# datavisorgaohui/kube-scheduler-simulator

Hardware: AMD Instinct MI355X
Metric: pod x node filter+score evals/sec (pods scheduled/sec in extra) (higher is better)
Workload: dtype int64/f64; 1 GPU; C2: 5000 nodes x 10000 pods, default profile, sequential, pct=100; nodes=5000, pods=10000, parallelism=scenario x1, percentage_of_nodes_to_score=100

## Files before the change

kube-scheduler-simulator_amd/csrc/kss_simple.cuh:

```cuda
#pragma once
#include "kss_fastmath.cuh"
#include "kss_sched.cuh"

namespace kss {

#define KSS_GLOBAL __attribute__((address_space(1)))
template <class T>
__device__ __forceinline__ KSS_GLOBAL T* gp(T* p) {
  return (KSS_GLOBAL T*)p;
}

template <class T>
__device__ __forceinline__ T ld_ag(const T* p) {
  return __hip_atomic_load(gp(p), __ATOMIC_RELAXED, __HIP_MEMORY_SCOPE_AGENT);
}
template <class T>
__device__ __forceinline__ T ld_ag(KSS_GLOBAL const T* p) {
  return __hip_atomic_load(p, __ATOMIC_RELAXED, __HIP_MEMORY_SCOPE_AGENT);
}
template <class T>
__device__ __forceinline__ void st_ag(T* p, T v) {
  __hip_atomic_store(gp(p), v, __ATOMIC_RELAXED, __HIP_MEMORY_SCOPE_AGENT);
}

// ... 1655 lines not shown
      if (sp && tid == 0) sp[1] = wall_clock64();
      best = wave_max_key(best, kb, c.node_base);
      if (sp && tid == 0) sp[2] = wall_clock64();
    } else {
      if (k >= k0) {
        if (keys) {
          for (int s = tid; s < own; s += nt) {
            const SVal e = cv_get(L, s == sub_s ? sub_h : s);
            const long long key = simple_key(prof, e, scored, max_tt, rtt, max_na, rna, (uint32_t)(c.node_base + lo + s));
            bool kept = true;
            if (WIN && wcs >= 0) {
              const int n = lo + s, seg = (n >= wsl ? 0 : W) + w;
              kept = seg < wcs || (seg == wcs && n < wd);
            }
            best = (e.f == 0 && kept && key > best) ? key : best;
          }
        }
        if (sp && tid == 0) sp[1] = wall_clock64();
        long long b[1] = {best};
        const int op[1] = {OP_MAX};
        block_red(H, parity, b, op);
        parity ^= 1;
        best = b[0];
        if (sp && tid == 0) sp[2] = wall_clock64();
      }
    }
    cand = best ? (int)(0xFFFFFFFFu - (uint32_t)(unsigned long long)best) - c.node_base - lo : -1;
    const SPod& qn = L.ring[(k + 1) % RING];
    const int sln = (k + 1) % RING;
    if constexpr (WIN) {
      if (k >= k0 && wcs >= 0) {
        wss = wcs % W;
        if (w == wss) wsx = wd;
        wsl = win_start(wss, wd);
      }
      uint32_t u[12];
      if (k + 1 < k1) {
        if constexpr (PW) simple_pass_a_pw_win<DEF>(prof, qn, pk, L, sln, own, pwv, cand, lo, wsl, u);
        else simple_pass_a_win<DEF>(prof, qn, pk, L, sln, own, cand, lo, wsl, u);
      } else {
#pragma unroll
        for (int i = 0; i < 12; i++) u[i] = 0;
      }
      if (sp && tid == 0) sp[3] = wall_clock64();
      if (!simple_sync_win<PW>(H, parity, best, u, W, w, ++epoch, gran, X, err, per, c.node_base, lo, own, pk, k >= k0, L,
                               kb, k_find, wsl, pwv, R, wd, wcs, sp, prefetch_idle))
        return;
    } else if constexpr (PW) {
      uint32_t u[6];
      if (k + 1 < k1) {
        simple_pass_a_pw<DEF>(prof, qn, pk, L, sln, own, pwv, cand, u);
      } else {
#pragma unroll
        for (int i = 0; i < 6; i++) u[i] = 0;
      }
      if (sp && tid == 0) sp[3] = wall_clock64();
      if (!simple_sync_pw(H, parity, best, u, W, w, ++epoch, gran, X, err, per, c.node_base, lo, own, pk, k >= k0, L, kb,
                          R, sp, prefetch_idle))
        return;
    } else {
      if (k + 1 < k1) {
        simple_pass_a<DEF>(prof, qn, pk, L, sln, own, cand, st);
      } else {
#pragma unroll
        for (int i = 0; i < 6; i++) st[i] = 0;
      }
      if (sp && tid == 0) sp[3] = wall_clock64();
      if (!simple_sync(H, parity, best, st, W, w, ++epoch, gran, X, err, per, c.node_base, kb, R, sp)) return;
    }
    if (sp && tid == 0) sp[5] = wall_clock64();
    if (k >= k0) {
      const long long K = R[0];
      const int x = K ? (int)(0xFFFFFFFFu - (uint32_t)(unsigned long long)K) - c.node_base : -1;
      const bool won = x >= lo && x < hi;
      sub_s = won ? x - lo : -1;
      sub_h = PW ? cap + (won ? (x - lo) / max(pwv, 1) : 0) : cap;
      if (!PW && !WIN && won && tid < 64) simple_commit_lanes(L, pk, x - lo, tid);
    }
    if (!defer_out) ring_store();
    if (k >= k0 && w == X.w_off && tid == out_tid) {
      const long long K = R[0];
      const int x = K ? (int)(0xFFFFFFFFu - (uint32_t)(unsigned long long)K) - c.node_base : -1;
      pend.chosen = K ? x + c.node_base : -1;
      pend.n_feasible = (int)nf;
      pend.scored = (K && scored) ? 1 : 0;
      pend.status = pk.status != 0 ? (pk.status == KSS_PF_ERROR ? 3 : 2) : (nf == 0 ? 1 : 0);
      pend.best_total = pend.scored ? (int64_t)((unsigned long long)K >> 32) : 0;
      pend_k = k;
      if (!defer_out) store_pending();
    }
    if (sp && tid == 0) sp[6] = wall_clock64();
  }
  if (tid == out_tid) store_pending();
  if constexpr (WIN) {
    if (X.n <= 1) {
      if (cursor && w == wss && tid == 0) st_ag(cursor, (int32_t)wsx);
    } else {
      const size_t co = 2 * (size_t)W * SXW_VALS + 2 * SXW_E2;
      ++epoch;
      if (w == wss && tid == 0) xpub(X, gran, co, ((unsigned long long)epoch << 32) | (uint32_t)wsx);
      if (w == X.w_off && tid == 0) {
        long long t0_ = 0;
        for (unsigned spins = 0;; ++spins) {
          const unsigned long long g = __hip_atomic_load(gran + co, __ATOMIC_RELAXED, __HIP_MEMORY_SCOPE_AGENT);
          if ((g >> 32) == epoch) {
            if (cursor) st_ag(cursor, (int32_t)(uint32_t)g);
            break;
          }
          if (spin_expired(spins, t0_)) {
            H.abort = 1;
            err_raise(err, 1);
            break;
          }
          spin_pause();
        }
      }
    }
  }
  __syncthreads();
  if (WIN && X.n > 1 && H.abort) return;
  for (int s = tid; s < own; s += nt) {
    const int n = lo + s;
#pragma unroll
    for (int r = 0; r < 3; r++) st_ag(&c.requested[(size_t)r * N + n], (int64_t)L.r64[(3 + r) * cap + s]);
    st_ag(&c.nonzero[n], (int64_t)L.r64[6 * cap + s]);
    st_ag(&c.nonzero[N + n], (int64_t)L.r64[7 * cap + s]);
    st_ag(&c.pod_count[n], L.r32[s]);
    for (int i = 0; i < L.nsc; i++) st_ag(&c.requested[(size_t)(3 + i) * N + n], L.sc[(size_t)(L.nsc + i) * cap + s]);
  }
  handoff_release();
}

constexpr int SXF_VALS = 4;
constexpr int SXF_LOADS = 8;
constexpr int SXF_MAX_E = 64 * SXF_LOADS / SXF_VALS;
static_assert(PW_LANES < 256, "granule 1 packs a wave's feasible counts in 8 bits");

__host__ __device__ constexpr int flat_entry(int gl, int per, int N, int nwave) {
  const int sh = gl / per, lo = sh * per;
  const int own = (N - lo < per ? N - lo : per);
  const int pwv = (own + nwave - 1) / nwave;
  return sh * nwave + (gl - lo) / pwv;
}
__host__ __device__ constexpr uint32_t flat_entry_range(int e, int per, int N, int W, int nwave) {
  const int sh = e / nwave, v = e - sh * nwave;
  if (sh >= W) return 0u;
  const int lo = sh * per;
  const int own = N - lo < 0 ? 0 : (N - lo < per ? N - lo : per);
  const int pwv = (own + nwave - 1) / nwave;
  const int a = v * pwv < own ? v * pwv : own, b = a + pwv < own ? a + pwv : own;
  return ((uint32_t)(lo + a) << 8) | (uint32_t)(b - a);
}
__host__ __device__ constexpr bool flat_range_holds(uint32_t r, int gl) {
  return (uint32_t)(gl - (int)(r >> 8)) < (r & 0xFFu);
}
__host__ __device__ constexpr bool flat_ranges_agree(int N, int W, int nwave) {
  const int per = (N + W - 1) / W;
  for (int gl = 0; gl < N; gl++)
    for (int e = 0; e < W * nwave; e++)
      if (flat_range_holds(flat_entry_range(e, per, N, W, nwave), gl) != (e == flat_entry(gl, per, N, nwave))) return false;
  for (int e = 0; e < W * nwave; e++)
    if (flat_range_holds(flat_entry_range(e, per, N, W, nwave), -1)) return false;
  return true;
}
static_assert(flat_ranges_agree(377, 3, 2) && flat_ranges_agree(378, 3, 2) && flat_ranges_agree(3, 3, 3) &&
                  flat_ranges_agree(10, 2, 3) && flat_ranges_agree(9, 2, 3) && flat_ranges_agree(5, 4, 2) &&
                  flat_ranges_agree(128, 64, 2) && flat_ranges_agree(1007, 2, 8),
              "flat_entry_range: the lanes' ranges are flat_entry's mapping");
static_assert(flat_entry(376, 126, 377, 2) == 5 && flat_entry(314, 126, 377, 2) == 4 && flat_entry(315, 126, 377, 2) == 5 &&
                  flat_entry(251, 126, 377, 2) == 3 && flat_entry(252, 126, 377, 2) == 4,
              "flat_entry: last shard one node short");
static_assert(flat_entry(0, 1, 3, 3) == 0 && flat_entry(1, 1, 3, 3) == 3 && flat_entry(2, 1, 3, 3) == 6,
              "flat_entry: shards of one node");
static_assert(flat_entry(1, 5, 10, 3) == 0 && flat_entry(2, 5, 10, 3) == 1 && flat_entry(4, 5, 10, 3) == 2 &&
                  flat_entry(5, 5, 10, 3) == 3 && flat_entry(9, 5, 10, 3) == 5,
              "flat_entry: own not divisible by nwave");
static_assert(flat_entry(8, 5, 9, 3) == 4 && flat_entry(6, 5, 9, 3) == 3, "flat_entry: short last shard, empty last wave");

template <typename Idle>
__device__ __forceinline__ bool simple_sync_flat(SimpleHdr& H, int& parity, long long wbest, uint32_t (&u)[6], int W,
                                                 int w, unsigned epoch, unsigned long long* gran, const XPeers& X,
                                                 int* err, int node_base, int kb, const uint32_t (&er)[SXF_LOADS],
                                                 long long (&R)[4], KSS_GLOBAL unsigned long long* sp, Idle&& idle) {
  wave_red_stats_pw(u);
  const int lane = threadIdx.x & 63, wave = threadIdx.x >> 6, nw = blockDim.x >> 6;
  const int E = W * nw;
  const unsigned long long tag = (unsigned long long)epoch << 32;
  if (sp && threadIdx.x == 0) sp[7] = wall_clock64();
  if (lane < SXF_VALS) {
    uint32_t x = key_compress(wbest, kb, node_base);
    x = lane == 1 ? (u[0] | (u[1] << 8) | (u[3] << 16) | (u[4] << 24)) : x;
    x = lane == 2 ? u[2] : x;
    x = lane == 3 ? u[5] : x;
    xpub(X, gran, ((size_t)(epoch & 1) * E + (size_t)w * nw + wave) * SXF_VALS + lane, tag | x);
  }
  if (sp && threadIdx.x == 0) sp[4] = wall_clock64();
  if (sp && (threadIdx.x == 64 || threadIdx.x == 128)) sp[9 + (threadIdx.x >> 6)] = wall_clock64();
  if (lane == 0) H.red[parity][wave][0] = wbest;
  lds_barrier();
  if (sp && threadIdx.x == 0) sp[8] = wall_clock64();
  idle();
  if (wave == 0) {
    if (sp && lane == 0) sp[15] = wall_clock64();
    const int G = SXF_VALS * E, nld = (G + 63) >> 6;
    const unsigned long long* base = gran + (size_t)(epoch & 1) * G;
    uint32_t got[SXF_LOADS];
    bool done = false;
    long long t0_ = 0;
    for (unsigned spins = 0;; ++spins) {
      bool ok = true;
      unsigned long long g[SXF_LOADS];
#pragma unroll
      for (int i = 0; i < SXF_LOADS; i++) {
        g[i] = tag;
        if (i < nld) {
          const int idx = i * 64 + lane;
          g[i] = __hip_atomic_load(base + (idx < G ? idx : 0), __ATOMIC_RELAXED, __HIP_MEMORY_SCOPE_AGENT);
        }
      }
#pragma unroll
      for (int i = 0; i < SXF_LOADS; i++) {
        ok &= (g[i] >> 32) == epoch;
        got[i] = i * 64 + lane < G ? (uint32_t)g[i] : 0u;
      }
      if (__all(ok)) {
        done = true;
        break;
      }
      if (spin_expired(spins, t0_)) break;
      spin_pause();
    }
    if (!done) {
      if (lane == 0) {
        H.abort = 1;
        err_raise(err, 1);
      }
    } else {
      const int field = lane & 3;
      uint32_t k = 0;
#pragma unroll
      for (int i = 0; i < SXF_LOADS; i++) k = max(k, got[i]);
      k = field == 0 ? k : 0u;
#define KSS_KSTEP(CTRL, ROWS) k = max(k, (uint32_t)__builtin_amdgcn_update_dpp(0, (int)k, CTRL, ROWS, 0xF, false))
      KSS_KSTEP(0xB1, 0xF);
      KSS_KSTEP(0x4E, 0xF);
      KSS_KSTEP(0x141, 0xF);
      KSS_KSTEP(0x140, 0xF);
      KSS_KSTEP(0x142, 0xA);
      KSS_KSTEP(0x143, 0xC);
#undef KSS_KSTEP
      k = (uint32_t)__builtin_amdgcn_readlane((int)k, 63);
      const long long best = key_expand(k, kb, node_base);
      const int gl = k ? (int)(((1u << kb) - 1u) - (k & ((1u << kb) - 1u))) : -1;
      uint32_t nf = 0, tt = 0, na = 0;
#pragma unroll
      for (int i = 0; i < SXF_LOADS; i++) {
        const bool h1 = flat_range_holds(er[i], gl);
        const uint32_t v = got[i];
        const uint32_t b = h1 ? v >> 16 : v;
        nf += field == 1 ? (b & 0xFFu) : 0u;
        tt = max(tt, field == 1 ? ((b >> 8) & 0xFFu) : 0u);
        na = max(na, (field == 2 && !h1) || (field == 3 && h1) ? v : 0u);
      }
#define KSS_FSTEP(CTRL, ROWS)                                                                      \
  {                                                                                                \
    const uint32_t a_ = (uint32_t)__builtin_amdgcn_update_dpp(0, (int)nf, CTRL, ROWS, 0xF, false); \
    const uint32_t b_ = (uint32_t)__builtin_amdgcn_update_dpp(0, (int)tt, CTRL, ROWS, 0xF, false); \
    const uint32_t c_ = (uint32_t)__builtin_amdgcn_update_dpp(0, (int)na, CTRL, ROWS, 0xF, false); \
    nf += a_;                                                                                      \
    tt = max(tt, b_);                                                                              \
    na = max(na, c_);                                                                              \
  }
      KSS_FSTEP(0xB1, 0xF)
      KSS_FSTEP(0x4E, 0xF)
      KSS_FSTEP(0x141, 0xF)
      KSS_FSTEP(0x140, 0xF)
      KSS_FSTEP(0x142, 0xA)
      KSS_FSTEP(0x143, 0xC)
#undef KSS_FSTEP
      if (lane == 63) {
        H.res[0] = best;
        H.res[1] = nf;
        H.res[2] = tt;
        H.res[3] = na;
      }
    }
  }
  parity ^= 1;
  lds_barrier();
  if (H.abort) return false;
#pragma unroll
  for (int i = 0; i < 4; i++) R[i] = H.res[i];
  return true;
}

template <bool FLAT>
__device__ __forceinline__ void simple_schedule_tab(DevCluster c, const SPod* __restrict__ spods,
                                                    const uint32_t* __restrict__ stat, int k0, int k1, int n_pods,
                                                    int32_t* chosen, PodMeta* meta, int W, int w, int cap,
                                                    unsigned long long* gran, const XPeers& X, unsigned epoch0, int* err,
                                                    unsigned long long* stamps, long long* smem, int n_shapes) {
  constexpr kss_profile prof = default_profile_c();
  constexpr int PD = 3;
  constexpr int NQ = (int)(sizeof(SPod) / 16);
  const int tid = threadIdx.x, nt = blockDim.x;
  SimpleHdr& H = *reinterpret_cast<SimpleHdr*>(smem);
  const SimpleShard L = shard_view(reinterpret_cast<uint8_t*>(smem) + sizeof(SimpleHdr), cap, 0);
  const ShapeTab TB = shape_tab_view(reinterpret_cast<uint8_t*>(smem), cap, n_shapes);
  const size_t N = (size_t)c.N;
  const int per = (c.N + W - 1) / W;
  const int lo = min(c.N, w * per), hi = min(c.N, lo + per), own = hi - lo;
  if (k1 <= k0) return;
  const int nwave = nt >> 6, lane = tid & 63, wv = tid >> 6;
  const int pwv = (own + nwave - 1) / nwave;
  const int s = wv * pwv + lane;
  const bool mine = lane < pwv && s < own;
  handoff_acquire();
  for (int i = tid; i < own; i += nt) {
    const int n = lo + i;
#pragma unroll
    for (int k = 0; k < 3; k++) {
      const int64_t A = c.alloc[k * N + n];
      L.r64[k * cap + i] = (double)A;
      L.r64[(3 + k) * cap + i] = (double)ld_ag(&c.requested[k * N + n]);
      L.inv[k * cap + i] = A > 0 ? 1.0 / (double)A : 0.0;
    }
    L.r64[6 * cap + i] = (double)ld_ag(&c.nonzero[n]);
    L.r64[7 * cap + i] = (double)ld_ag(&c.nonzero[N + n]);
    L.r32[i] = ld_ag(&c.pod_count[n]);
    L.r32[cap + i] = c.allowed_pods[n];
    for (int d = 0; d < PD && k0 + d < k1; d++) L.st[((k0 + d) % RING) * cap + i] = ld_ag(&stat[(size_t)d * N + lo + i]);
  }
  for (int i = tid; i < min(k1 - k0, PD) * NQ; i += nt) {
    const int j = k0 + i / NQ;
    reinterpret_cast<uint4*>(L.ring + j % RING)[i % NQ] = reinterpret_cast<const uint4*>(spods + j)[i % NQ];
  }
  for (int j = tid; j < n_shapes; j += nt) {
    const SPod& r = spods[min(max(spods[j].shape_rep, 0), n_pods - 1)];
    SShape d;
#pragma unroll
    for (int i = 0; i < 3; i++) d.fit_req[i] = r.fit_req[i];
#pragma unroll
    for (int i = 0; i < 2; i++) {
      d.snz[i] = r.snz[i];
      d.sreq[i] = r.sreq[i];
    }
    d.flags = r.flags;
    d.pad = 0;
    uint64_t dw[SSHAPE_WORDS];
    __builtin_memcpy(dw, &d, sizeof(SShape));
#pragma unroll
    for (int i = 0; i < SSHAPE_WORDS; i++) TB.shp[i * n_shapes + j] = dw[i];
  }
  if (tid == 0) H.abort = 0;
  __syncthreads();
  if (mine) {
    const DynRow r = shard_row(L, s);
    for (int j = 0; j < n_shapes; j++) TB.T[j * TB.ts + s] = shape_pack(dyn_eval_def(shape_get(TB, j), 0u, r));
  }
  __syncthreads();

  KSS_GLOBAL const uint32_t* gstat = gp(stat);
  KSS_GLOBAL const uint4* gspod = gp(reinterpret_cast<const uint4*>(spods));
  KSS_GLOBAL unsigned long long* gstamps = gp(stamps);
  long long R[4] = {0, 0, 0, 0};
  constexpr int out_tid = 64;
  PodMeta pend{};
  int pend_k = -1;
  auto store_pending = [&]() {
    if (pend_k < 0) return;
    if (chosen) gp(chosen)[pend_k] = pend.chosen;
    if (meta) {
      KSS_GLOBAL PodMeta* mm = gp(meta) + pend_k;
      mm->chosen = pend.chosen;
      mm->n_feasible = pend.n_feasible;
      mm->scored = pend.scored;
      mm->status = pend.status;
      mm->best_total = pend.best_total;
    }
    pend_k = -1;
  };
  int parity = 0;
  unsigned epoch = epoch0;
  const int kb = key_bits(prof, c.N);
  const int pf_w0 = nwave >= 3 ? nwave - 1 : 1;
  const bool pf_wave = __builtin_amdgcn_readfirstlane(tid >> 6) >= pf_w0;
  uint4 pfq = make_uint4(0, 0, 0, 0);
  uint32_t pfw[PF_MAX];
#pragma unroll
  for (int j = 0; j < PF_MAX; j++) pfw[j] = 0;
  const int pf_lane = tid - 64 * pf_w0, pf_n = nt - 64 * pf_w0;
  const int pf_per = (own + pf_n - 1) / pf_n;
  const int idle_n = 64 * (nwave - 1), jobs = nwave * n_shapes;
  const int job0 = tid - 64;
  const int v0 = job0 >= 0 ? job0 / n_shapes : 0, j0 = job0 >= 0 ? job0 % n_shapes : 0;
  int ck = 0, cn = min(max(L.ring[k0 % RING].shape, 0), n_shapes - 1), cnn = 0;
  uint32_t er[SXF_LOADS] = {};
  if constexpr (FLAT) {
#pragma unroll
    for (int i = 0; i < SXF_LOADS; i++) er[i] = flat_entry_range(i * 16 + (lane >> 2), per, c.N, W, nwave);
  }
  for (int k = k0 - 1; k < k1; k++) {
    KSS_GLOBAL unsigned long long* sp = (stamps && k >= k0 && k - k0 < KSS_NSTAMP_PODS / 2)
                                            ? gstamps + (size_t)w * 8 * KSS_NSTAMP_PODS + (size_t)(k - k0) * 16
                                            : nullptr;
    if (sp && tid == 0) sp[0] = wall_clock64();
    if (sp && tid == 64) sp[9] = wall_clock64();
    const SPod& pk = L.ring[(k + RING) % RING];
    const SPod& qn = L.ring[(k + 1) % RING];
    const int slk = (k + RING) % RING, sln = (k + 1) % RING;
    if (k + 2 < k1) cnn = min(max(L.ring[(k + 2) % RING].shape, 0), n_shapes - 1);
    const bool pf_on = pf_wave && k >= k0 && k + PD < k1 && own > 0;
    if (pf_on) {
      KSS_GLOBAL const uint4& src = gspod[(size_t)(k + PD) * NQ + min(pf_lane, NQ - 1)];
      pfq = make_uint4(src.x, src.y, src.z, src.w);
#pragma unroll
      for (int j = 0; j < PF_MAX; j++)
        if (j < pf_per) pfw[j] = ld_ag(&gstat[(size_t)(k + PD - k0) * N + lo + min(j * pf_n + pf_lane, own - 1)]);
    }
    const bool refresh_on = k >= k0 && k + 1 < k1;
    const long long nf = R[1];
    const int max_tt = (int)R[2], max_na = (int)R[3];
    const bool scored = nf > 1;
    const bool keys = k >= k0 && pk.status == 0 && nf > 0;
    const float rtt = __builtin_amdgcn_rcpf((float)max(max_tt, 1));
    const float rna = __builtin_amdgcn_rcpf((float)max(max_na, 1));
    long long best = 0;
    if (keys && mine) {
      const uint32_t t = TB.T[ck * TB.ts + s], wd = L.st[slk * cap + s];
      const SVal e{sw_code(wd), sw_tt(wd), sw_na(wd), (int)((t >> 8) & 0xFFu), (int)(t & 0xFFu)};
      const long long key = simple_key(prof, e, scored, max_tt, rtt, max_na, rna, (uint32_t)(c.node_base + lo + s));
      best = (e.f == 0 && (t & ST_FITS)) ? key : 0;
    }
    if (sp && tid == 0) sp[1] = wall_clock64();
    best = wave_max_key(best, kb, c.node_base);
    if (sp && tid == 0) sp[2] = wall_clock64();
    const int cand = best ? (int)(0xFFFFFFFFu - (uint32_t)(unsigned long long)best) - c.node_base - lo : -1;
    uint32_t u[6] = {0, 0, 0, 0, 0, 0};
    if (k + 1 < k1) {
      const bool extra = lane == pwv && cand >= 0;
      if (mine || extra) {
        const int ns = extra ? cand : s;
        const uint32_t wd = L.st[sln * cap + ns];
        bool ok;
        if (extra) {
          bool bad = (int64_t)L.r32[ns] + 2 > (int64_t)L.r32[cap + ns];
          bool sh = false;
#pragma unroll
          for (int i = 0; i < 3; i++)
            sh |= qn.fit_req[i] > L.r64[i * cap + ns] - (L.r64[(3 + i) * cap + ns] + pk.creq[i]);
          bad |= !(qn.flags & SP_ALLZERO) & sh;
          ok = !bad;
        } else {
          ok = (TB.T[cn * TB.ts + s] & ST_FITS) != 0;
        }
        ok &= sw_code(wd) == 0;
        const bool c0 = ok && !extra, c1 = ok && (extra || s != cand);
        const uint32_t tt = (uint32_t)sw_tt(wd), na = (uint32_t)sw_na(wd);
        u[0] = c0 ? 1u : 0u;
        u[1] = c0 ? tt : 0u;
        u[2] = c0 ? na : 0u;
        u[3] = c1 ? 1u : 0u;
        u[4] = c1 ? tt : 0u;
        u[5] = c1 ? na : 0u;
      }
    }
    if (sp && tid == 0) sp[3] = wall_clock64();
    auto idle = [&]() {
      if (refresh_on && keys && wv > 0) {
        for (int job = job0, rd = 0; job < jobs; job += idle_n, rd++) {
          const int v = rd == 0 ? v0 : job / n_shapes, j = rd == 0 ? j0 : job % n_shapes;
          const long long kv = H.red[parity][v][0];
          if (kv == 0) continue;
          const int cs = (int)(0xFFFFFFFFu - (uint32_t)(unsigned long long)kv) - c.node_base - lo;
          DynRow r = shard_row(L, cs);
          add_commit(r, pk);
          TB.pnd[v * KSS_MAX_SHAPES + j] = shape_pack(dyn_eval_def(shape_get(TB, j), 0u, r));
        }
        if (sp && (tid == 64 || tid == 128)) sp[11 + (tid >> 6)] = wall_clock64();
      }
      if (pf_on) {
        reinterpret_cast<uint4*>(L.ring + (k + PD) % RING)[min(pf_lane, NQ - 1)] = pfq;
#pragma unroll
        for (int j = 0; j < PF_MAX; j++)
          if (j < pf_per) L.st[((k + PD) % RING) * cap + min(j * pf_n + pf_lane, own - 1)] = pfw[j];
      }
      if (tid == out_tid) store_pending();
    };
    bool synced;
    if constexpr (FLAT)
      synced = simple_sync_flat(H, parity, best, u, W, w, ++epoch, gran, X, err, c.node_base, kb, er, R, sp, idle);
    else
      synced = simple_sync_pw(H, parity, best, u, W, w, ++epoch, gran, X, err, per, c.node_base, lo, own, pk, false, L, kb,
                              R, sp, idle);
    if (!synced) return;
    if (sp && tid == 0) sp[5] = wall_clock64();
    if (k >= k0) {
      const long long K = R[0];
      const int x = K ? (int)(0xFFFFFFFFu - (uint32_t)(unsigned long long)K) - c.node_base : -1;
      if (x >= lo && x < hi && (x - lo) / max(pwv, 1) == wv) {
        simple_commit_lanes(L, pk, x - lo, lane);
        if (refresh_on && lane < n_shapes) TB.T[lane * TB.ts + (x - lo)] = TB.pnd[wv * KSS_MAX_SHAPES + lane];
      }
      if (w == X.w_off && tid == out_tid) {
        pend.chosen = K ? x + c.node_base : -1;
        pend.n_feasible = (int)nf;
        pend.scored = (K && scored) ? 1 : 0;
        pend.status = pk.status != 0 ? (pk.status == KSS_PF_ERROR ? 3 : 2) : (nf == 0 ? 1 : 0);
        pend.best_total = pend.scored ? (int64_t)((unsigned long long)K >> 32) : 0;
        pend_k = k;
      }
    }
    ck = cn;
    cn = cnn;
    if (sp && tid == 0) sp[6] = wall_clock64();
  }
  if (tid == out_tid) store_pending();
  __syncthreads();
  for (int i = tid; i < own; i += nt) {
    const int n = lo + i;
#pragma unroll
    for (int r = 0; r < 3; r++) st_ag(&c.requested[(size_t)r * N + n], (int64_t)L.r64[(3 + r) * cap + i]);
    st_ag(&c.nonzero[n], (int64_t)L.r64[6 * cap + i]);
    st_ag(&c.nonzero[N + n], (int64_t)L.r64[7 * cap + i]);
    st_ag(&c.pod_count[n], L.r32[i]);
  }
  handoff_release();
}

__device__ __forceinline__ void simple_counts(const DevCluster& c, const SPod* __restrict__ spods,
                                              const int32_t* __restrict__ ints, const int32_t* __restrict__ chosen,
                                              int k) {
  const int x = chosen[k] - c.node_base;
  if (x < 0 || x >= c.N) return;
  const SPod& q = spods[k];
  const size_t N = (size_t)c.N;
  if (q.cls >= 0) atomicAdd(&c.class_count[(size_t)q.cls * N + x], 1);
  for (int i = 0; i < q.own_len; i++) atomicAdd(&c.term_count[(size_t)ints[q.own_off + i] * N + x], 1);
}

}
```

Baseline: 1.737 billion evals/s.

## Stage next pod's LDS operands into registers during sync idle window

Per-node table entries, status words and pod request fields for the next iteration are now loaded from LDS into registers inside the idle lambda that runs while waiting on the cross-workgroup sync. The critical path between syncs then starts from registers rather than LDS reads. The global prefetch is split into a load issued one iteration earlier (PD+1) and an LDS store one iteration later, so global latency is hidden across a sync. This adds register pressure and requires patching the staged values for the committed node, which makes correctness depend on ring-slot reuse invariants.

```diff
diff --git a/kube-scheduler-simulator_amd/csrc/kss_simple.cuh b/kube-scheduler-simulator_amd/csrc/kss_simple.cuh
--- a/kube-scheduler-simulator_amd/csrc/kss_simple.cuh
+++ b/kube-scheduler-simulator_amd/csrc/kss_simple.cuh
@@ -1981,6 +1981,8 @@
                                                     unsigned long long* stamps, long long* smem, int n_shapes) {
   constexpr kss_profile prof = default_profile_c();
   constexpr int PD = 3;
+  constexpr int PD_TAB = PD + 1;
+  static_assert(PD_TAB == RING, "window k stores ring slot (k - 1) % RING: no reader left (see Staging)");
   constexpr int NQ = (int)(sizeof(SPod) / 16);
   const int tid = threadIdx.x, nt = blockDim.x;
   SimpleHdr& H = *reinterpret_cast<SimpleHdr*>(smem);
@@ -2073,12 +2075,31 @@
   const int idle_n = 64 * (nwave - 1), jobs = nwave * n_shapes;
   const int job0 = tid - 64;
   const int v0 = job0 >= 0 ? job0 / n_shapes : 0, j0 = job0 >= 0 ? job0 % n_shapes : 0;
-  int ck = 0, cn = min(max(L.ring[k0 % RING].shape, 0), n_shapes - 1), cnn = 0;
+  int cn = min(max(L.ring[k0 % RING].shape, 0), n_shapes - 1), cnn = 0;
   uint32_t er[SXF_LOADS] = {};
   if constexpr (FLAT) {
 #pragma unroll
     for (int i = 0; i < SXF_LOADS; i++) er[i] = flat_entry_range(i * 16 + (lane >> 2), per, c.N, W, nwave);
   }
+  uint32_t sa_t = 0, sa_w = 0, sb_t = 0, sb_w = 0;
+  int32_t s_status = 0, s_flags = 0;
+  double s_creq[3] = {0.0, 0.0, 0.0}, s_fit[3] = {0.0, 0.0, 0.0};
+  const int ss = mine ? s : 0;
+  auto stage = [&](int kk, int ca, int cb) {
+    const int ra = (kk + RING) % RING, rb = (kk + 1) % RING;
+    sa_t = TB.T[ca * TB.ts + ss];
+    sa_w = L.st[ra * cap + ss];
+    sb_t = TB.T[cb * TB.ts + ss];
+    sb_w = L.st[rb * cap + ss];
+    s_status = L.ring[ra].status;
+    s_flags = L.ring[rb].flags;
+#pragma unroll
+    for (int i = 0; i < 3; i++) {
+      s_creq[i] = L.ring[ra].creq[i];
+      s_fit[i] = L.ring[rb].fit_req[i];
+    }
+  };
+  stage(k0 - 1, 0, cn);
   for (int k = k0 - 1; k < k1; k++) {
     KSS_GLOBAL unsigned long long* sp = (stamps && k >= k0 && k - k0 < KSS_NSTAMP_PODS / 2)
                                             ? gstamps + (size_t)w * 8 * KSS_NSTAMP_PODS + (size_t)(k - k0) * 16
@@ -2086,30 +2107,25 @@
     if (sp && tid == 0) sp[0] = wall_clock64();
     if (sp && tid == 64) sp[9] = wall_clock64();
     const SPod& pk = L.ring[(k + RING) % RING];
-    const SPod& qn = L.ring[(k + 1) % RING];
-    const int slk = (k + RING) % RING, sln = (k + 1) % RING;
+    const int sln = (k + 1) % RING;
     if (k + 2 < k1) cnn = min(max(L.ring[(k + 2) % RING].shape, 0), n_shapes - 1);
-    const bool pf_on = pf_wave && k >= k0 && k + PD < k1 && own > 0;
-    if (pf_on) {
-      KSS_GLOBAL const uint4& src = gspod[(size_t)(k + PD) * NQ + min(pf_lane, NQ - 1)];
-      pfq = make_uint4(src.x, src.y, src.z, src.w);
-#pragma unroll
-      for (int j = 0; j < PF_MAX; j++)
-        if (j < pf_per) pfw[j] = ld_ag(&gstat[(size_t)(k + PD - k0) * N + lo + min(j * pf_n + pf_lane, own - 1)]);
-    }
+    const bool pf_ld = pf_wave && k + PD_TAB < k1 && own > 0;
+    const bool pf_st = pf_wave && k >= k0 && k + PD < k1 && own > 0;
     const bool refresh_on = k >= k0 && k + 1 < k1;
+    const uint32_t a_t = sa_t, a_w = sa_w, b_t = sb_t, b_w = sb_w;
+    const int32_t k_status = s_status, n_flags = s_flags;
+    const double k_creq[3] = {s_creq[0], s_creq[1], s_creq[2]}, n_fit[3] = {s_fit[0], s_fit[1], s_fit[2]};
     const long long nf = R[1];
     const int max_tt = (int)R[2], max_na = (int)R[3];
     const bool scored = nf > 1;
-    const bool keys = k >= k0 && pk.status == 0 && nf > 0;
+    const bool keys = k >= k0 && k_status == 0 && nf > 0;
     const float rtt = __builtin_amdgcn_rcpf((float)max(max_tt, 1));
     const float rna = __builtin_amdgcn_rcpf((float)max(max_na, 1));
     long long best = 0;
-    if (keys && mine) {
-      const uint32_t t = TB.T[ck * TB.ts + s], wd = L.st[slk * cap + s];
-      const SVal e{sw_code(wd), sw_tt(wd), sw_na(wd), (int)((t >> 8) & 0xFFu), (int)(t & 0xFFu)};
+    {
+      const SVal e{sw_code(a_w), sw_tt(a_w), sw_na(a_w), (int)((a_t >> 8) & 0xFFu), (int)(a_t & 0xFFu)};
       const long long key = simple_key(prof, e, scored, max_tt, rtt, max_na, rna, (uint32_t)(c.node_base + lo + s));
-      best = (e.f == 0 && (t & ST_FITS)) ? key : 0;
+      best = (keys && mine && e.f == 0 && (a_t & ST_FITS)) ? key : 0;
     }
     if (sp && tid == 0) sp[1] = wall_clock64();
     best = wave_max_key(best, kb, c.node_base);
@@ -2118,31 +2134,34 @@
     uint32_t u[6] = {0, 0, 0, 0, 0, 0};
     if (k + 1 < k1) {
       const bool extra = lane == pwv && cand >= 0;
-      if (mine || extra) {
-        const int ns = extra ? cand : s;
-        const uint32_t wd = L.st[sln * cap + ns];
-        bool ok;
-        if (extra) {
-          bool bad = (int64_t)L.r32[ns] + 2 > (int64_t)L.r32[cap + ns];
-          bool sh = false;
-#pragma unroll
-          for (int i = 0; i < 3; i++)
-            sh |= qn.fit_req[i] > L.r64[i * cap + ns] - (L.r64[(3 + i) * cap + ns] + pk.creq[i]);
-          bad |= !(qn.flags & SP_ALLZERO) & sh;
-          ok = !bad;
-        } else {
-          ok = (TB.T[cn * TB.ts + s] & ST_FITS) != 0;
+      bool ok = mine && (b_t & ST_FITS) != 0;
+      uint32_t wd = b_w;
+      if (extra) {
+        const int ns = cand;
+        wd = L.st[sln * cap + ns];
+        const int32_t pods = L.r32[ns], allowed = L.r32[cap + ns];
+        double al[3], rq[3];
+#pragma unroll
+        for (int i = 0; i < 3; i++) {
+          al[i] = L.r64[i * cap + ns];
+          rq[i] = L.r64[(3 + i) * cap + ns];
         }
-        ok &= sw_code(wd) == 0;
-        const bool c0 = ok && !extra, c1 = ok && (extra || s != cand);
-        const uint32_t tt = (uint32_t)sw_tt(wd), na = (uint32_t)sw_na(wd);
-        u[0] = c0 ? 1u : 0u;
-        u[1] = c0 ? tt : 0u;
-        u[2] = c0 ? na : 0u;
-        u[3] = c1 ? 1u : 0u;
-        u[4] = c1 ? tt : 0u;
-        u[5] = c1 ? na : 0u;
-      }
+        bool bad = (int64_t)pods + 2 > (int64_t)allowed;
+        bool sh = false;
+#pragma unroll
+        for (int i = 0; i < 3; i++) sh |= n_fit[i] > al[i] - (rq[i] + k_creq[i]);
+        bad |= !(n_flags & SP_ALLZERO) & sh;
+        ok = !bad;
+      }
+      ok &= sw_code(wd) == 0;
+      const bool c0 = ok && !extra, c1 = ok && (extra || s != cand);
+      const uint32_t tt = (uint32_t)sw_tt(wd), na = (uint32_t)sw_na(wd);
+      u[0] = c0 ? 1u : 0u;
+      u[1] = c0 ? tt : 0u;
+      u[2] = c0 ? na : 0u;
+      u[3] = c1 ? 1u : 0u;
+      u[4] = c1 ? tt : 0u;
+      u[5] = c1 ? na : 0u;
     }
     if (sp && tid == 0) sp[3] = wall_clock64();
     auto idle = [&]() {
@@ -2158,11 +2177,19 @@
         }
         if (sp && (tid == 64 || tid == 128)) sp[11 + (tid >> 6)] = wall_clock64();
       }
-      if (pf_on) {
+      stage(k + 1, cn, cnn);
+      if (pf_st) {
         reinterpret_cast<uint4*>(L.ring + (k + PD) % RING)[min(pf_lane, NQ - 1)] = pfq;
 #pragma unroll
         for (int j = 0; j < PF_MAX; j++)
           if (j < pf_per) L.st[((k + PD) % RING) * cap + min(j * pf_n + pf_lane, own - 1)] = pfw[j];
+      }
+      if (pf_ld) {
+        KSS_GLOBAL const uint4& src = gspod[(size_t)(k + PD_TAB) * NQ + min(pf_lane, NQ - 1)];
+        pfq = make_uint4(src.x, src.y, src.z, src.w);
+#pragma unroll
+        for (int j = 0; j < PF_MAX; j++)
+          if (j < pf_per) pfw[j] = ld_ag(&gstat[(size_t)(k + PD_TAB - k0) * N + lo + min(j * pf_n + pf_lane, own - 1)]);
       }
       if (tid == out_tid) store_pending();
     };
@@ -2178,6 +2205,10 @@
       const long long K = R[0];
       const int x = K ? (int)(0xFFFFFFFFu - (uint32_t)(unsigned long long)K) - c.node_base : -1;
       if (x >= lo && x < hi && (x - lo) / max(pwv, 1) == wv) {
+        if (refresh_on && s == x - lo) {
+          sa_t = TB.pnd[wv * KSS_MAX_SHAPES + cn];
+          sb_t = TB.pnd[wv * KSS_MAX_SHAPES + cnn];
+        }
         simple_commit_lanes(L, pk, x - lo, lane);
         if (refresh_on && lane < n_shapes) TB.T[lane * TB.ts + (x - lo)] = TB.pnd[wv * KSS_MAX_SHAPES + lane];
       }
@@ -2185,12 +2216,11 @@
         pend.chosen = K ? x + c.node_base : -1;
         pend.n_feasible = (int)nf;
         pend.scored = (K && scored) ? 1 : 0;
-        pend.status = pk.status != 0 ? (pk.status == KSS_PF_ERROR ? 3 : 2) : (nf == 0 ? 1 : 0);
+        pend.status = k_status != 0 ? (k_status == KSS_PF_ERROR ? 3 : 2) : (nf == 0 ? 1 : 0);
         pend.best_total = pend.scored ? (int64_t)((unsigned long long)K >> 32) : 0;
         pend_k = k;
       }
     }
-    ck = cn;
     cn = cnn;
     if (sp && tid == 0) sp[6] = wall_clock64();
   }
```

Measured after the change: 1.945 billion evals/s (median of 6 runs). 12.0% higher.
